# vacp2p/zerokit

Measured on AMD Instinct MI355X. Metric: RLN Groth16 proofs/sec (BN254, h=20), higher is better.
Workload: dtype u32 limbs (256-bit Montgomery integers, BN254 Fr/Fq; 8x32 and 9x29 forms)

## Files before the change

zerokit_amd/csrc/fq29.h:

```cpp
#pragma once
#include <hip/hip_runtime.h>
#include <stdint.h>

#include "curve.h"
#include "fq29_constants.h"

namespace rlnamd {

template <class C, class Mont>
struct F29 {
  uint32_t v[9];

  static constexpr uint32_t M = (1u << 29) - 1;

  static __device__ __forceinline__ F29 from_const(const uint32_t (&c)[9]) {
    F29 r;
#pragma unroll
    for (int j = 0; j < 9; j++) r.v[j] = c[j];
    return r;
  }
  static __device__ __forceinline__ F29 zero() {
    F29 r;
#pragma unroll
    for (int j = 0; j < 9; j++) r.v[j] = 0;
// ... 175 lines not shown
    const bool ge = borrow == 0;
    const uint32_t r0 = ge ? d[0] : v[0], r1 = ge ? d[1] : v[1], r2 = ge ? d[2] : v[2], r3 = ge ? d[3] : v[3],
                   r4 = ge ? d[4] : v[4], r5 = ge ? d[5] : v[5], r6 = ge ? d[6] : v[6], r7 = ge ? d[7] : v[7],
                   r8 = ge ? d[8] : v[8];
    Mont o;
    o.v[0] = r0 | (r1 << 29);
    o.v[1] = (r1 >> 3) | (r2 << 26);
    o.v[2] = (r2 >> 6) | (r3 << 23);
    o.v[3] = (r3 >> 9) | (r4 << 20);
    o.v[4] = (r4 >> 12) | (r5 << 17);
    o.v[5] = (r5 >> 15) | (r6 << 14);
    o.v[6] = (r6 >> 18) | (r7 << 11);
    o.v[7] = (r7 >> 21) | (r8 << 8);
    return o;
  }
  static __device__ __forceinline__ F29 from_fq(const Mont& a) {
    return mul(slice(a), from_const(C::FROM_FQ));
  }
  __device__ __forceinline__ Mont to_fq() const {
    return mul(*this, from_const(C::TO_FQ)).pack_reduced();
  }
  static __device__ __forceinline__ Mont mul_mont(const Mont& a, const F29& w29) { return mul(slice(a), w29).pack_reduced(); }
};

using Fq29 = F29<Fq29C, Fq>;
using Fr29 = F29<Fr29C, Fr>;

struct G1Affine29 {
  uint32_t x[8], y[8];
  __device__ __forceinline__ bool is_inf() const {
// ... 48 lines not shown
  __device__ __forceinline__ void store_xyzz(G1XYZZ* dst) const { *dst = to_xyzz(); }
  static __device__ __forceinline__ G1Acc29 load_xyzz(const G1XYZZ* src) { return from_xyzz(*src); }
  __device__ __forceinline__ void store_lds(G1Acc29* dst) const { *dst = *this; }

  static __device__ __forceinline__ G1Acc29 inf() { return {Fq29::zero(), Fq29::zero(), Fq29::zero(), Fq29::zero()}; }
  __device__ __forceinline__ bool is_inf() const { return ZZ.limbs_all_zero(); }

  __device__ __forceinline__ G1XYZZ to_xyzz() const {
    if (is_inf()) return G1XYZZ::inf();
    return {X.to_fq(), Y.to_fq(), ZZ.to_fq(), ZZZ.to_fq()};
  }
  static __device__ __forceinline__ G1Acc29 from_xyzz(const G1XYZZ& p) {
    if (p.is_inf()) return inf();
    return {Fq29::from_fq(p.X), Fq29::from_fq(p.Y), Fq29::from_fq(p.ZZ), Fq29::from_fq(p.ZZZ)};
  }

  static __device__ __forceinline__ G1Acc29 dbl_affine(const Fq29& x, const Fq29& py) {
    Fq29 U;
#pragma unroll
    for (int j = 0; j < 9; j++) U.v[j] = 2 * py.v[j];
    Fq29 V = Fq29::sqr(U);
    Fq29 W = Fq29::mul(U, V);
    Fq29 S = Fq29::mul(x, V);
    Fq29 x2 = Fq29::sqr(x);
    Fq29 Mm;
#pragma unroll
    for (int j = 0; j < 9; j++) Mm.v[j] = 3 * x2.v[j];
    Mm.normalize();
    Fq29 M2 = Fq29::sqr(Mm);
    Fq29 X3;
#pragma unroll
    for (int j = 0; j < 9; j++) X3.v[j] = M2.v[j] + Fq29C::K4T[j] - 2 * S.v[j];
    X3.normalize();
    Fq29 D = Fq29::sub(S, Fq29C::K6, X3);
    Fq29 nY = Fq29::neg_lazy(Fq29C::K4, py);
    return {X3, Fq29::dot2(Mm, D, nY, W), V, W};
  }

  __device__ __forceinline__ void madd(const G1Affine29& e, bool negate) {
    const Fq29 px = unpack29(e.x);
    Fq29 py = unpack29(e.y);
    if (negate) py = Fq29::neg_lazy(Fq29C::K2, py);
    if (is_inf()) {
      X = px;
      Y = py;
      Y.normalize();
      ZZ = Fq29::from_const(Fq29C::ONE);
      ZZZ = ZZ;
      return;
    }
    const Fq29 kX = Fq29::neg_lazy(Fq29C::K6, X);
// ... 12 lines not shown
    Fq29 PP = Fq29::sqr(P);
    ZZ = Fq29::mul(ZZ, PP);
    Fq29 Q = Fq29::mul(X, PP);
    Fq29 PPP = Fq29::mul(P, PP);
    ZZZ = Fq29::mul(ZZZ, PPP);
    Fq29 kT;
#pragma unroll
    for (int j = 0; j < 9; j++) kT.v[j] = Fq29C::K4T[j] - (PPP.v[j] + 2 * Q.v[j]);
    X = Fq29::sqr_add(R, &kT);
    Fq29 D;
#pragma unroll
    for (int j = 0; j < 9; j++) D.v[j] = Q.v[j] + Fq29C::K6[j] - X.v[j];
    Y = Fq29::dot2(R, D, nY, PPP);
  }

  __device__ __forceinline__ void add(const G1Acc29& o) {
    if (o.is_inf()) return;
    if (is_inf()) {
      *this = o;
      return;
    }
    const Fq29 U1 = Fq29::mul(X, o.ZZ), U2 = Fq29::mul(o.X, ZZ);
    const Fq29 S1 = Fq29::mul(Y, o.ZZZ), S2 = Fq29::mul(o.Y, ZZZ);
    const Fq29 P = Fq29::sub(U2, Fq29C::K2, U1), R = Fq29::sub(S2, Fq29C::K2, S1);
    if (P.is_zero_mod_q()) {
      add_same_x(this, &o);
      return;
    }
    const Fq29 PP = Fq29::sqr(P);
    ZZ = Fq29::mul(Fq29::mul(ZZ, o.ZZ), PP);
    const Fq29 Q = Fq29::mul(U1, PP);
    const Fq29 PPP = Fq29::mul(P, PP);
    ZZZ = Fq29::mul(Fq29::mul(ZZZ, o.ZZZ), PPP);
    Fq29 kT;
#pragma unroll
    for (int j = 0; j < 9; j++) kT.v[j] = Fq29C::K4T[j] - (PPP.v[j] + 2 * Q.v[j]);
    X = Fq29::sqr_add(R, &kT);
    Fq29 D;
#pragma unroll
    for (int j = 0; j < 9; j++) D.v[j] = Q.v[j] + Fq29C::K6[j] - X.v[j];
    const Fq29 nS1 = Fq29::neg_lazy(Fq29C::K4, S1);
// ... 230 lines not shown
  Fq2_29 X, Y, ZZ, ZZZ;
  static constexpr uint32_t LPP = O::LPP;
  static __device__ __forceinline__ G2AccT inf() {
    Fq2_29 z{Fq29::zero(), Fq29::zero()};
    return {z, z, z, z};
  }
  __device__ __forceinline__ bool is_inf() const { return ZZ.c0.limbs_all_zero() && ZZ.c1.limbs_all_zero(); }
  __device__ __forceinline__ G2XYZZ to_xyzz() const {
    if (is_inf()) return G2XYZZ::inf();
    return {X.to_fq2(), Y.to_fq2(), ZZ.to_fq2(), ZZZ.to_fq2()};
  }
  static __device__ __forceinline__ G2AccT from_xyzz(const G2XYZZ& p) {
    if (p.is_inf()) return inf();
    return {Fq2_29::from_fq2(p.X), Fq2_29::from_fq2(p.Y), Fq2_29::from_fq2(p.ZZ), Fq2_29::from_fq2(p.ZZZ)};
  }
  __device__ __forceinline__ void store_xyzz(G2XYZZ* dst) const {
    if (LPP == 1) {
      *dst = to_xyzz();
      return;
    }
    const bool o = Fq2PairOps::odd(), z = is_inf();
    const Fq2_29* const c[4] = {&X, &Y, &ZZ, &ZZZ};
    Fq2* const d[4] = {&dst->X, &dst->Y, &dst->ZZ, &dst->ZZZ};
#pragma unroll
    for (int k = 0; k < 4; k++) {
      const Fq v = z ? Fq::zero() : Fq2PairOps::pick(o, c[k]->c1, c[k]->c0).to_fq();
      *(o ? &d[k]->c1 : &d[k]->c0) = v;
    }
  }
  __device__ __forceinline__ void store_lds(G2AccT* dst) const {
// ... 44 lines not shown
#pragma unroll
    for (int j = 0; j < 9; j++) {
      X3.c0.v[j] = M2.c0.v[j] + Fq29C::K4T[j] - 2 * S.c0.v[j];
      X3.c1.v[j] = M2.c1.v[j] + Fq29C::K4T[j] - 2 * S.c1.v[j];
    }
    X3.c0.normalize();
    X3.c1.normalize();
    Fq2_29 D = Fq2_29::sub(S, Fq29C::K6, X3);
    Fq29 nM1 = Fq29::neg_lazy(Fq29C::K8, Mm.c1);
    Fq29 ny0 = Fq29::neg_lazy(Fq29C::K4, y.c0);
    Fq29 ny1 = Fq29::neg_lazy(Fq29C::K4, y.c1);
    Fq29 y0 = Fq29::dot4<true>(Mm.c0, D.c0, nM1, D.c1, W.c0, ny0, W.c1, y.c1);
    Fq29 y1 = Fq29::dot4<true>(Mm.c0, D.c1, Mm.c1, D.c0, W.c0, ny1, W.c1, ny0);
    return {X3, {y0, y1}, V, W};
  }

  __device__ __forceinline__ void madd(const G2Affine29& e, bool negate) {
    const Fq2_29 px{unpack29(e.x0), unpack29(e.x1)};
    Fq2_29 py{unpack29(e.y0), unpack29(e.y1)};
    if (negate) {
      py.c0 = Fq29::neg_lazy(Fq29C::K2, py.c0);
      py.c1 = Fq29::neg_lazy(Fq29C::K2, py.c1);
      py.c0.normalize();
      py.c1.normalize();
    }
    if (is_inf()) {
      X = px;
      Y = py;
      ZZ = {Fq29::from_const(Fq29C::ONE), Fq29::zero()};
      ZZZ = ZZ;
// ... 11 lines not shown
    ZZ = O::mul(ZZ, PP);
    Fq2_29 Q = O::mul(X, PP);
    Fq2_29 PPP = O::mul(P, PP);
    ZZZ = O::mul(ZZZ, PPP);
    Fq2_29 kT;
#pragma unroll
    for (int j = 0; j < 9; j++) {
      kT.c0.v[j] = Fq29C::K4T[j] - (PPP.c0.v[j] + 2 * Q.c0.v[j]);
      kT.c1.v[j] = Fq29C::K4T[j] - (PPP.c1.v[j] + 2 * Q.c1.v[j]);
    }
    X = O::sqr_add(R, kT);
    Fq2_29 D = Fq2_29::sub(Q, Fq29C::K6, X);
    Y = O::rd_minus_st(R, D, nY, Y, PPP);
  }

  __device__ __forceinline__ void add(const G2AccT* o) {
    if (o->is_inf()) return;
    if (is_inf()) {
      *this = *o;
      return;
    }
    Fq2_29 U1, P, S1, R;
    {
      const Fq2_29 oZZ = o->ZZ, oX = o->X;
      U1 = O::mul(X, oZZ);
      const Fq2_29 U2 = O::mul(oX, ZZ);
      P = Fq2_29::sub(U2, Fq29C::K2, U1);
    }
    asm volatile("" ::: "memory");
    {
      const Fq2_29 oZZZ = o->ZZZ, oY = o->Y;
      S1 = O::mul(Y, oZZZ);
      const Fq2_29 S2 = O::mul(oY, ZZZ);
      R = Fq2_29::sub(S2, Fq29C::K2, S1);
    }
    if (P.is_zero_mod_q()) {
      add_same_x(this, o);
      return;
    }
    asm volatile("" ::: "memory");
    {
      const Fq2_29 oZZ = o->ZZ;
      ZZ = O::mul(ZZ, oZZ);
    }
    {
      const Fq2_29 oZZZ = o->ZZZ;
      ZZZ = O::mul(ZZZ, oZZZ);
    }
    asm volatile("" ::: "memory");
    const Fq2_29 PP = O::sqr(P);
    ZZ = O::mul(ZZ, PP);
    const Fq2_29 Q = O::mul(U1, PP);
// ... 25 lines not shown
```

zerokit_amd/csrc/prover.hip:

```cpp
#include "prover.h"

#include <fcntl.h>
#include <stdlib.h>
#include <string.h>
#include <sys/stat.h>
#include <time.h>
#include <unistd.h>

#include <algorithm>
#include <atomic>
#include <chrono>
#include <deque>
#include <mutex>
#include <thread>

#include "prover_kernels.h"
#include "prover_plan.h"
#include "fq29.h"
#include "glv.h"
#include "pairing.h"
#include "poseidon.h"
#include "witness_ops.h"
#include "witness_lanes.h"
#include "witness_sched.h"
// ... 1343 lines not shown
  hipStream_t sA2 = big ? D.st[role[ROLE_QUOTIENT]] : !early ? D.sA2 : sh.g2_on_front ? D.sB2 : sA;
  const uint32_t pg = div_up(nb, 64);
  const uint32_t nbp = pg * 64;
  auto d2h = [&](void* host, const void* dev, size_t bytes, hipStream_t st) {
    if (!small && bytes % 16 == 0)
      hipLaunchKernelGGL(k_stage_in, dim3(div_up(bytes / 16, 64)), dim3(64), 0, st, (const uint4*)dev, (uint4*)host, (uint32_t)(bytes / 16));
    else
      RLN_HIP(hipMemcpyAsync(host, dev, bytes, hipMemcpyDeviceToHost, st));
  };
  auto walk1 = [&](hipStream_t st, const uint32_t* ids, uint32_t cnt) {
    if (!cnt) return;
    const uint32_t blocks = div_up(cnt, 8) * 8 * pg;
    if (!small) {
      const PairPlan pp{P1.prows.p, P1.prsid.p, P1.pchunks.p, P1.pout.p, P1.npchunks};
      const uint32_t pblocks = div_up(P1.npchunks, 8) * 8 * (2 * pg);
      hipLaunchKernelGGL((k_msm29<G1Acc29, G1Affine29, G1XYZZ, 4>), dim3(blocks + pblocks), dim3(64), 0, st, D.t1_29.p,
                         P1.rsid.p, P1.rows.p, P1.chunks.p, cnt, S.digits.p, S.part1.p, D.ws, dB, pg, D.nh, D.walk_clk.p, ids,
                         0u, pp);
    } else if (walk_lp) {
      hipLaunchKernelGGL((k_msm29<G1Acc29, G1Affine29, G1XYZZ, 4>), dim3(blocks), dim3(64), 0, st, D.t1_29.p, P1.rsid.p,
                         P1.rows.p, P1.chunks.p, cnt, S.digits.p, S.part1.p, D.ws, dB, pg, D.nh, nullptr, ids, PB);
    } else {
      hipLaunchKernelGGL((k_msm29<G1Acc29, G1Affine29, G1XYZZ, 2, true>), dim3(div_up(cnt, 64), nb), dim3(64), 0, st,
                         D.t1_29.p, P1.rsid.p, P1.rows.p, P1.chunks.p, cnt, S.digits.p, S.part1.p, D.ws, dB, PB, D.nh,
                         nullptr, ids);
    }
  };
  if (S.used) RLN_HIP(hipStreamWaitEvent(sA, S.free_event(), 0));
  if (streamed) {
    auto h2d = [&](void* dst, const uint8_t* src, size_t bytes) {
      hipLaunchKernelGGL(k_stage_in, dim3(div_up(bytes / 16, 64)), dim3(64), 0, sA, (const uint4*)src, (uint4*)dst,
// ... 168 lines not shown
  MARK(11, s2);
  if (P2.nchunks) {
    uint32_t blocks = div_up(P2.nchunks, 8) * 8 * pg;
    if (walk_lp)
      hipLaunchKernelGGL((k_msm29<G2Acc29, G2Affine29, G2XYZZ, 2>), dim3(blocks), dim3(64), 0, s2, D.t2_29.p, P2.rsid.p,
                         P2.rows.p, P2.chunks.p, P2.nchunks, S.digits2.p, S.part2.p, D.ws2, dB, pg, D.nh, nullptr, nullptr, PB);
    else if (tiny)
      hipLaunchKernelGGL((k_msm29<G2AccPair29, G2Affine29, G2XYZZ, 1, true>), dim3(div_up(2 * P2.nchunks, 64), nb), dim3(64), 0, s2,
                         D.t2_29.p, P2.rsid.p, P2.rows.p, P2.chunks.p, P2.nchunks, S.digits2.p, S.part2.p, D.ws2, dB, PB, D.nh,
                         nullptr);
    else if (small)
      hipLaunchKernelGGL((k_msm29<G2Acc29, G2Affine29, G2XYZZ, 1, true>), dim3(div_up(P2.nchunks, 64), nb), dim3(64), 0, s2,
                         D.t2_29.p, P2.rsid.p, P2.rows.p, P2.chunks.p, P2.nchunks, S.digits2.p, S.part2.p, D.ws2, dB, PB, D.nh,
                         nullptr);
    else
      hipLaunchKernelGGL((k_msm29<G2Acc29, G2Affine29, G2XYZZ, 2>), dim3(blocks), dim3(64), 0, s2, D.t2_29.p, P2.rsid.p,
                         P2.rows.p, P2.chunks.p, P2.nchunks, S.digits2.p, S.part2.p, D.ws2, dB, pg, D.nh,
                         D.walk_clk.p ? D.walk_clk.p + 2 : nullptr);
  }
  MARK(8, s2);
  if (!compact) RLN_HIP(hipEventRecord(S.evB, sB1));
  RLN_HIP(hipEventRecord(S.evB2, s2));
  hipStream_t sV = compact ? s2 : D.sV;
  hipStream_t sC = big ? D.st[role[ROLE_SUMS2]] : D.sC;
  if (S.used && !compact) {
    RLN_HIP(hipStreamWaitEvent(sC, S.free_event(), 0));
    RLN_HIP(hipStreamWaitEvent(sV, S.free_event(), 0));
  }
  if (!values_front) {
    if (streamed && !compact) RLN_HIP(hipStreamWaitEvent(sV, S.evU, 0));
    MARK(0, sV);
// ... 73 lines not shown
      hipLaunchKernelGGL(k_fin_out_ac, dim3(pg), dim3(64), 0, sAC, S.sums1.p, S.prod.p, S.affA.p, S.coords.p, S.comp.p, B, nbp);
    if (lone) {
      RLN_HIP(hipEventRecord(S.evA, sAC));
      RLN_HIP(hipStreamWaitEvent(sF, S.evA, 0));
    }
    RLN_HIP(hipStreamWaitEvent(sF, S.evV, 0));
  } else {
    if (tiny_partial) {
      sum2(s2);
      RLN_HIP(hipEventRecord(S.evB2, s2));
    }
    if (!values_front) RLN_HIP(hipEventRecord(S.evV, sV));
    if (compact) {
      hipStream_t sS1 = D.st[role[ROLE_SUMS1]];
      if (P1.ngroups)
        hipLaunchKernelGGL(k_sum_ranges<Fq>, dim3(pg, P1.ngroups), dim3(64), 0, sS1, S.part1.p, P1.groups.p, P1.ngroups,
                           S.grp1.p, B, nbp);
      hipLaunchKernelGGL(k_sum_ranges<Fq>, dim3(pg, P1.nseg), dim3(64), 0, sS1, S.grp1.p, P1.segs.p, P1.nseg, S.sums1.p, B, nbp);
      RLN_HIP(hipEventRecord(S.evB, sS1));
      MARK(9, sC);
      if (P2.ngroups)
        hipLaunchKernelGGL(k_sum_ranges<Fq2>, dim3(pg, P2.ngroups), dim3(64), 0, sC, S.part2.p, P2.groups.p, P2.ngroups,
                           S.grp2.p, B, nbp);
      hipLaunchKernelGGL(k_sum_ranges<Fq2>, dim3(pg, P2.nseg), dim3(64), 0, sC, S.grp2.p, P2.segs.p, P2.nseg, S.sums2.p, B, nbp);
      RLN_HIP(hipStreamWaitEvent(sC, S.evB, 0));
      RLN_HIP(hipStreamWaitEvent(sC, S.evV, 0));
    } else {
      RLN_HIP(hipStreamWaitEvent(sC, S.evV, 0));
      RLN_HIP(hipStreamWaitEvent(sC, S.evB, 0));
      if (tiny_partial) sum1(sC, {0, 1, 2, 3, 4, 5});
      RLN_HIP(hipStreamWaitEvent(sC, S.evB2, 0));
      MARK(9, sC);
    }
  }
  if (early || tiny_partial || compact) {
  } else if (small) {
    sum1(sC, {0, 1, 2, 3, 4, 5});
    sum2(sC);
  } else {
    if (P1.ngroups)
      hipLaunchKernelGGL(k_sum_ranges<Fq>, dim3(pg, P1.ngroups), dim3(64), 0, sC, S.part1.p, P1.groups.p, P1.ngroups,
                         S.grp1.p, B, nbp);
    if (P2.ngroups)
      hipLaunchKernelGGL(k_sum_ranges<Fq2>, dim3(pg, P2.ngroups), dim3(64), 0, sC, S.part2.p, P2.groups.p, P2.ngroups,
                         S.grp2.p, B, nbp);
    hipLaunchKernelGGL(k_sum_ranges<Fq>, dim3(pg, P1.nseg), dim3(64), 0, sC, S.grp1.p, P1.segs.p, P1.nseg, S.sums1.p, B, nbp);
    hipLaunchKernelGGL(k_sum_ranges<Fq2>, dim3(pg, P2.nseg), dim3(64), 0, sC, S.grp2.p, P2.segs.p, P2.nseg, S.sums2.p, B, nbp);
  }
  if (!early)
    hipLaunchKernelGGL(k_glv_fold, dim3(pg, 4), dim3(64), 0, sC, S.sums1.p, S.sums2.p, 3u, B, nbp, all4);
  if (mode == PROVE_PARTIAL) {
    hipLaunchKernelGGL(k_partial_out, dim3(pg, 4), dim3(64), 0, sC, S.sums1.p, S.sums2.p, S.pp_out.p, B, nbp);
    RLN_HIP(hipGetLastError());
    d2h(S.h_pp, S.pp_out.p, n * 320, sC);
  } else {
    if (!early) {
      if (mode == PROVE_FINISH)
        hipLaunchKernelGGL(k_add_partial, dim3(pg, 4), dim3(64), 0, sC, S.sums1.p, S.sums2.p, pp_p, B, nbp, all4, (const G1XYZZ*)nullptr);
      hipLaunchKernelGGL(k_fin_affine, dim3(pg, 3), dim3(64), 0, sC, S.sums1.p, S.sums2.p, S.affA.p, S.affB1.p,
                         S.affB2.p, B, nbp, all3);
      hipLaunchKernelGGL(k_fin_smul, dim3(pg, 2), dim3(64), 0, sC, S.affA.p, S.affB1.p, rs_p, S.tbl.p, S.prod.p, B,
                         nbp);
// ... 206 lines not shown
```

zerokit_amd/csrc/prover_kernels.h:

```cpp
#pragma once
#include <hip/hip_runtime.h>
#include <stdint.h>

#include <initializer_list>

#include "fq29.h"
#include "poseidon.h"
#include "prover.h"
#include "prover_desc.h"
#include "prover_plan.h"
#include "walk29.h"
#include "witness_ops.h"

namespace rlnamd {

struct CsrView {
  const uint32_t* ptr;
  const uint32_t* col;
  const Fr* coef;
};

struct TaskSel {
  uint8_t id[8];
};
// ... 41 lines not shown
__global__ void __launch_bounds__(256) k_ntt_mid(Fr* __restrict__ data, const Fr* __restrict__ tw_i,
                                                 const Fr* __restrict__ tw_f, int logn, const Fr* __restrict__ scale,
                                                 uint32_t B, uint32_t nb);
template <bool DIF>
__global__ void __launch_bounds__(256) k_ntt_edge(Fr* __restrict__ data, const Fr* __restrict__ tw, int logn, uint32_t B,
                                                  uint32_t nb);
__global__ void __launch_bounds__(256) k_recode(const Fr* __restrict__ V, const uint32_t* __restrict__ sig2node,
                                                uint32_t ns, const Fr* H, uint32_t n,
                                                const uint32_t* __restrict__ rs, WinSched ws1, WinSched ws2,
                                                int16_t* __restrict__ dig1, int16_t* __restrict__ dig2, uint32_t B,
                                                uint32_t nb, uint32_t part, uint32_t lg, uint32_t hq, uint32_t dB);

template <class A, class E>
__global__ void __launch_bounds__(256) k_table_to29(const A* __restrict__ src, E* __restrict__ dst, size_t n, uint32_t stride,
                                                    uint32_t k0, uint32_t npaired);
template <class F>
__global__ void __launch_bounds__(64) k_sum_ranges(const XYZZ<F>* __restrict__ src, const ChunkDesc* __restrict__ ranges,
                                                   uint32_t nranges, XYZZ<F>* __restrict__ dst, uint32_t B, uint32_t nb);
template <class F, class Acc>
__global__ void __launch_bounds__(SUM_TREE_LANES) k_sum_tree(const XYZZ<F>* __restrict__ part, const ChunkDesc* __restrict__ segchunks,
                                                  XYZZ<F>* __restrict__ dst, uint32_t B, uint32_t PB, TaskSel sel);
template <class F, class Acc>
__global__ void __launch_bounds__(SUM_TREE_LANES) k_sum_blocks(const XYZZ<F>* __restrict__ part, const ChunkDesc* __restrict__ segchunks,
                                                    const ChunkDesc* __restrict__ segblocks, XYZZ<F>* __restrict__ dst, uint32_t PB,
                                                    TaskSel sel);
__global__ void __launch_bounds__(64) k_glv_fold(G1XYZZ* __restrict__ sums1, G2XYZZ* __restrict__ sums2, uint32_t nseg1,
                                                 uint32_t B, uint32_t nb, TaskSel sel);
template <class F>
__global__ void __launch_bounds__(64) k_table_build(const Affine<F>* __restrict__ pts, uint32_t npts, WinSched ws,
                                                    Affine<F>* __restrict__ table, F* __restrict__ scratch);

// ... 61 lines not shown
```

zerokit_amd/csrc/prover_walks.hip:

```cpp
#include "prover_kernels.h"

#include "glv.h"
#include "walk29_impl.h"

namespace rlnamd {

template <class A, class E>
__global__ void __launch_bounds__(256) k_table_to29(const A* __restrict__ src, E* __restrict__ dst, size_t n, uint32_t stride,
                                                    uint32_t k0, uint32_t npaired) {
  size_t t = (size_t)blockIdx.x * 256 + threadIdx.x;
  if (t >= n) return;
  const uint32_t kl = (uint32_t)(t / stride), x = (uint32_t)(t % stride), k = k0 + kl;
  size_t o = t;
  if (k < npaired) o = (size_t)(kl & ~1u) * stride + 2 * (size_t)x + (kl & 1u);
  dst[o] = to_table29(src[t]);
}

template <class F>
__global__ void __launch_bounds__(64) k_sum_ranges(const XYZZ<F>* __restrict__ src, const ChunkDesc* __restrict__ ranges,
                                                   uint32_t nranges, XYZZ<F>* __restrict__ dst, uint32_t B, uint32_t nb) {
  __builtin_amdgcn_s_setprio(3);
  uint32_t p = blockIdx.x * 64 + threadIdx.x;
  uint32_t r = blockIdx.y;
  if (p >= nb || r >= nranges) return;
  ChunkDesc cd = ranges[r];
  XYZZ<F> acc = XYZZ<F>::inf();
  for (uint32_t i = cd.pt_begin; i < cd.pt_end; i++) acc.add(src[(size_t)i * B + p]);
  dst[(size_t)r * B + p] = acc;
}

template <class F> struct Acc29Of;
template <> struct Acc29Of<Fq> { typedef G1Acc29 type; };
template <> struct Acc29Of<Fq2> { typedef G2Acc29 type; };
extern __shared__ uint4 sum_tree_lds[];

template <class F, class Acc>
__global__ void __launch_bounds__(SUM_TREE_LANES) k_sum_tree(const XYZZ<F>* __restrict__ part, const ChunkDesc* __restrict__ segchunks,
                                                  XYZZ<F>* __restrict__ dst, uint32_t B, uint32_t PB, TaskSel sel) {
  constexpr uint32_t NP = SUM_TREE_LANES / Acc::LPP;
  Acc* sh = reinterpret_cast<Acc*>(sum_tree_lds);
  __builtin_amdgcn_s_setprio(3);
  const uint32_t p = blockIdx.x, sgi = sel.id[blockIdx.y], l = threadIdx.x / Acc::LPP;
  const ChunkDesc cd = segchunks[sgi];
  Acc acc = Acc::inf();
  for (uint32_t i = cd.pt_begin + l; i < cd.pt_end; i += NP) acc.add(Acc::load_xyzz(&part[(size_t)i * PB + p]));
#pragma unroll 1
  for (uint32_t stride = NP / 2; stride >= 1; stride >>= 1) {
    if (l >= stride && l < 2 * stride) acc.store_lds(&sh[l - stride]);
// ... 108 lines not shown
        lam = (x2.dbl() + x2) * di;
        x3 = lam.sqr() - Pm.x.dbl();
        y3 = lam * (Pm.x - x3) - Pm.y;
      }
      inv = inv * den;
      row[m + i - 1] = {x3, y3};
    }
    __threadfence_block();
    __syncthreads();
  }
}


template __global__ void k_table_to29<G1Affine, G1Affine29>(const G1Affine* __restrict__ src, G1Affine29* __restrict__ dst, size_t n, uint32_t stride, uint32_t k0, uint32_t npaired);
template __global__ void k_table_to29<G2Affine, G2Affine29>(const G2Affine* __restrict__ src, G2Affine29* __restrict__ dst, size_t n, uint32_t stride, uint32_t k0, uint32_t npaired);
template __global__ void k_sum_ranges<Fq>(const XYZZ<Fq>* __restrict__ src, const ChunkDesc* __restrict__ ranges, uint32_t nranges, XYZZ<Fq>* __restrict__ dst, uint32_t B, uint32_t nb);
template __global__ void k_sum_ranges<Fq2>(const XYZZ<Fq2>* __restrict__ src, const ChunkDesc* __restrict__ ranges, uint32_t nranges, XYZZ<Fq2>* __restrict__ dst, uint32_t B, uint32_t nb);
template __global__ void k_sum_tree<Fq, G1Acc29>(const XYZZ<Fq>* __restrict__ part, const ChunkDesc* __restrict__ segchunks, XYZZ<Fq>* __restrict__ dst, uint32_t B, uint32_t PB, TaskSel sel);
template __global__ void k_sum_tree<Fq, G1AccPair29>(const XYZZ<Fq>* __restrict__ part, const ChunkDesc* __restrict__ segchunks, XYZZ<Fq>* __restrict__ dst, uint32_t B, uint32_t PB, TaskSel sel);
template __global__ void k_sum_tree<Fq2, G2Acc29>(const XYZZ<Fq2>* __restrict__ part, const ChunkDesc* __restrict__ segchunks, XYZZ<Fq2>* __restrict__ dst, uint32_t B, uint32_t PB, TaskSel sel);
template __global__ void k_sum_blocks<Fq, G1Acc29>(const XYZZ<Fq>* __restrict__ part, const ChunkDesc* __restrict__ segchunks, const ChunkDesc* __restrict__ segblocks, XYZZ<Fq>* __restrict__ dst, uint32_t PB, TaskSel sel);
template __global__ void k_sum_blocks<Fq, G1AccPair29>(const XYZZ<Fq>* __restrict__ part, const ChunkDesc* __restrict__ segchunks, const ChunkDesc* __restrict__ segblocks, XYZZ<Fq>* __restrict__ dst, uint32_t PB, TaskSel sel);
template __global__ void k_sum_blocks<Fq2, G2Acc29>(const XYZZ<Fq2>* __restrict__ part, const ChunkDesc* __restrict__ segchunks, const ChunkDesc* __restrict__ segblocks, XYZZ<Fq2>* __restrict__ dst, uint32_t PB, TaskSel sel);
template __global__ void k_sum_tree<Fq2, G2AccPair29>(const XYZZ<Fq2>* __restrict__ part, const ChunkDesc* __restrict__ segchunks, XYZZ<Fq2>* __restrict__ dst, uint32_t B, uint32_t PB, TaskSel sel);
template __global__ void k_sum_blocks<Fq2, G2AccPair29>(const XYZZ<Fq2>* __restrict__ part, const ChunkDesc* __restrict__ segchunks, const ChunkDesc* __restrict__ segblocks, XYZZ<Fq2>* __restrict__ dst, uint32_t PB, TaskSel sel);
template __global__ void k_table_build<Fq>(const Affine<Fq>* __restrict__ pts, uint32_t npts, WinSched ws, Affine<Fq>* __restrict__ table, Fq* __restrict__ scratch);
template __global__ void k_table_build<Fq2>(const Affine<Fq2>* __restrict__ pts, uint32_t npts, WinSched ws, Affine<Fq2>* __restrict__ table, Fq2* __restrict__ scratch);
template __global__ void k_msm29<G1Acc29, G1Affine29, G1XYZZ, 4, false>(const G1Affine29* __restrict__ table, const uint32_t* __restrict__ sid, const uint32_t* __restrict__ rows, const ChunkDesc* __restrict__ chunks, uint32_t nchunks, const int16_t* __restrict__ digits, G1XYZZ* __restrict__ part, WinSched ws, uint32_t B, uint32_t pgroups, uint32_t nh, unsigned long long* __restrict__ clk, const uint32_t* __restrict__ chunk_ids, uint32_t pstride, PairPlan pairs);
template __global__ void k_msm29<G1Acc29, G1Affine29, G1XYZZ, 2, true>(const G1Affine29* __restrict__ table, const uint32_t* __restrict__ sid, const uint32_t* __restrict__ rows, const ChunkDesc* __restrict__ chunks, uint32_t nchunks, const int16_t* __restrict__ digits, G1XYZZ* __restrict__ part, WinSched ws, uint32_t B, uint32_t pgroups, uint32_t nh, unsigned long long* __restrict__ clk, const uint32_t* __restrict__ chunk_ids, uint32_t pstride, PairPlan pairs);
template __global__ void k_msm29<G2Acc29, G2Affine29, G2XYZZ, 2, false>(const G2Affine29* __restrict__ table, const uint32_t* __restrict__ sid, const uint32_t* __restrict__ rows, const ChunkDesc* __restrict__ chunks, uint32_t nchunks, const int16_t* __restrict__ digits, G2XYZZ* __restrict__ part, WinSched ws, uint32_t B, uint32_t pgroups, uint32_t nh, unsigned long long* __restrict__ clk, const uint32_t* __restrict__ chunk_ids, uint32_t pstride, PairPlan pairs);
template __global__ void k_msm29<G2Acc29, G2Affine29, G2XYZZ, 1, true>(const G2Affine29* __restrict__ table, const uint32_t* __restrict__ sid, const uint32_t* __restrict__ rows, const ChunkDesc* __restrict__ chunks, uint32_t nchunks, const int16_t* __restrict__ digits, G2XYZZ* __restrict__ part, WinSched ws, uint32_t B, uint32_t pgroups, uint32_t nh, unsigned long long* __restrict__ clk, const uint32_t* __restrict__ chunk_ids, uint32_t pstride, PairPlan pairs);
template __global__ void k_msm29<G2AccPair29, G2Affine29, G2XYZZ, 1, true>(const G2Affine29* __restrict__ table, const uint32_t* __restrict__ sid, const uint32_t* __restrict__ rows, const ChunkDesc* __restrict__ chunks, uint32_t nchunks, const int16_t* __restrict__ digits, G2XYZZ* __restrict__ part, WinSched ws, uint32_t B, uint32_t pgroups, uint32_t nh, unsigned long long* __restrict__ clk, const uint32_t* __restrict__ chunk_ids, uint32_t pstride, PairPlan pairs);

}
```

zerokit_amd/csrc/walk29.h:

```cpp
#pragma once
#include <hip/hip_runtime.h>
#include <stdint.h>

#include "fq29.h"
#include "prover_desc.h"

namespace rlnamd {

template <class Entry>
__device__ __forceinline__ const Entry* row_base(const Entry* __restrict__ table, uint32_t roww, uint32_t stride, uint32_t* shift) {
  const uint32_t k = roww & ROW_INDEX, il = (roww >> 30) & 1u;
  *shift = il;
  return table + (size_t)(il ? (k & ~1u) : k) * stride + (il ? (k & 1u) : 0u);
}

struct PairPlan {
  const uint32_t* rows;
  const uint32_t* sid;
  const ChunkDesc* chunks;
  const uint32_t* out;
  uint32_t nchunks;
};

template <class Acc, class Entry, class Out, int WAVES, bool LANECHUNK = false>
__global__ void __launch_bounds__(64) __attribute__((amdgpu_waves_per_eu(WAVES, WAVES))) k_msm29(const Entry* __restrict__ table, const uint32_t* __restrict__ sid,
                                              const uint32_t* __restrict__ rows, const ChunkDesc* __restrict__ chunks,
                                              uint32_t nchunks, const int16_t* __restrict__ digits,
                                              Out* __restrict__ part, WinSched ws, uint32_t B, uint32_t pgroups,
                                              uint32_t nh, unsigned long long* __restrict__ clk,
                                              const uint32_t* __restrict__ chunk_ids = nullptr, uint32_t pstride = 0,
                                              PairPlan pairs = PairPlan{nullptr, nullptr, nullptr, nullptr, 0});

}
```

zerokit_amd/csrc/walk29_impl.h:

```cpp
#pragma once
#include "walk29.h"

namespace rlnamd {

template <class Acc, class Entry, class Out, int WAVES, bool LANECHUNK>
__global__ void __launch_bounds__(64) __attribute__((amdgpu_waves_per_eu(WAVES, WAVES))) k_msm29(const Entry* __restrict__ table, const uint32_t* __restrict__ sid,
                                              const uint32_t* __restrict__ rows, const ChunkDesc* __restrict__ chunks,
                                              uint32_t nchunks, const int16_t* __restrict__ digits,
                                              Out* __restrict__ part, WinSched ws, uint32_t B, uint32_t pgroups,
                                              uint32_t nh, unsigned long long* __restrict__ clk,
                                              const uint32_t* __restrict__ chunk_ids, uint32_t pstride, PairPlan pairs) {
  const unsigned long long c0 = clk ? clock64() : 0, w0 = clk ? wall_clock64() : 0;
  uint32_t L = blockIdx.x;
  const int W = ws.W;
  if (LANECHUNK) {
    const uint32_t idx = (L * 64 + threadIdx.x) / Acc::LPP, p = blockIdx.y;
    if (idx >= nchunks) return;
    const uint32_t chunk = chunk_ids ? chunk_ids[idx] : idx;
    const ChunkDesc cd = chunks[chunk];
    Acc acc = Acc::inf();
    struct Cur {
      uint32_t i, j;
    };
    auto adv = [&](Cur& c) {
// ... 55 lines not shown
#pragma unroll 1
  for (uint32_t i = cd.pt_begin; i < cd.pt_end; i++) {
    const uint32_t kk = R[i] + member;
    const int16_t* dg = digits + ((size_t)S[i] * nh + (kk >> 31)) * W * B + p;
    uint32_t sh;
    const Entry* row = row_base(table, kk, ws.stride, &sh);
#pragma unroll 1
    for (int j = 0; j < W; j++) {
      int d = dg[(size_t)j * B];
      if (d != 0) {
        uint32_t e = (uint32_t)(d < 0 ? -d : d) - 1;
        acc.madd(row[(size_t)(ws.ro[j] + e) << sh], d < 0);
      }
    }
  }
  part[(size_t)out_slot * (pstride ? pstride : B) + p] = acc.to_xyzz();
  if (clk && threadIdx.x == 0 && (L & 63) == 0) {
    atomicAdd(clk, clock64() - c0);
    atomicAdd(clk + 1, wall_clock64() - w0);
  }
}

}
```

Measured before the change: 23120.

## Hand off MSM partials in loose 29-bit Montgomery form to range-sum kernels

The MSM walk kernels now write bucket partials in a loosely reduced, packed 9x29-limb form instead of fully converting each coordinate back to canonical 8x32 Montgomery with a multiply. The range-sum kernels are reworked to accumulate with the 29-bit accumulator types, slicing the handoff form directly, and only the final segment pass converts to canonical XYZZ. This removes per-partial to_fq/from_fq multiplies and replaces 32-bit XYZZ adds with the faster 29-bit adds. The same-x case is handled inline with a new doubling routine. It relies on loose values fitting in 256 bits after a conditional 4q subtraction on X, and adds LDS staging for G2 operands.

```diff
diff --git a/zerokit_amd/csrc/fq29.h b/zerokit_amd/csrc/fq29.h
--- a/zerokit_amd/csrc/fq29.h
+++ b/zerokit_amd/csrc/fq29.h
@@ -213,6 +213,30 @@
     o.v[7] = (r7 >> 21) | (r8 << 8);
     return o;
   }
+  __device__ __forceinline__ Mont pack_loose() const {
+    Mont o;
+    o.v[0] = v[0] | (v[1] << 29);
+    o.v[1] = (v[1] >> 3) | (v[2] << 26);
+    o.v[2] = (v[2] >> 6) | (v[3] << 23);
+    o.v[3] = (v[3] >> 9) | (v[4] << 20);
+    o.v[4] = (v[4] >> 12) | (v[5] << 17);
+    o.v[5] = (v[5] >> 15) | (v[6] << 14);
+    o.v[6] = (v[6] >> 18) | (v[7] << 11);
+    o.v[7] = (v[7] >> 21) | (v[8] << 8);
+    return o;
+  }
+  __device__ __forceinline__ F29 minus_4q_if_above() const {
+    const bool above = v[8] > C::KP[4][8];
+    F29 r;
+    int32_t borrow = 0;
+#pragma unroll
+    for (int j = 0; j < 9; j++) {
+      const int32_t x = (int32_t)v[j] - (int32_t)(above ? C::KP[4][j] : 0u) + borrow;
+      r.v[j] = j < 8 ? (uint32_t)x & M : (uint32_t)x;
+      borrow = x >> 29;
+    }
+    return r;
+  }
   static __device__ __forceinline__ F29 from_fq(const Mont& a) {
     return mul(slice(a), from_const(C::FROM_FQ));
   }
@@ -291,6 +315,12 @@
     if (p.is_inf()) return inf();
     return {Fq29::from_fq(p.X), Fq29::from_fq(p.Y), Fq29::from_fq(p.ZZ), Fq29::from_fq(p.ZZZ)};
   }
+  __device__ __forceinline__ void store_handoff(G1XYZZ* dst) const {
+    *dst = {X.minus_4q_if_above().pack_loose(), Y.pack_loose(), ZZ.pack_loose(), ZZZ.pack_loose()};
+  }
+  static __device__ __forceinline__ G1Acc29 from_handoff(const G1XYZZ& p) {
+    return {Fq29::slice(p.X), Fq29::slice(p.Y), Fq29::slice(p.ZZ), Fq29::slice(p.ZZZ)};
+  }
 
   static __device__ __forceinline__ G1Acc29 dbl_affine(const Fq29& x, const Fq29& py) {
     Fq29 U;
@@ -312,6 +342,12 @@
     Fq29 D = Fq29::sub(S, Fq29C::K6, X3);
     Fq29 nY = Fq29::neg_lazy(Fq29C::K4, py);
     return {X3, Fq29::dot2(Mm, D, nY, W), V, W};
+  }
+  __device__ __forceinline__ G1Acc29 dbl() const {
+    G1Acc29 r = dbl_affine(X, Y);
+    r.ZZ = Fq29::mul(r.ZZ, ZZ);
+    r.ZZZ = Fq29::mul(r.ZZZ, ZZZ);
+    return r;
   }
 
   __device__ __forceinline__ void madd(const G1Affine29& e, bool negate) {
@@ -354,6 +390,7 @@
     Y = Fq29::dot2(R, D, nY, PPP);
   }
 
+  template <bool SAME_X_HERE = false>
   __device__ __forceinline__ void add(const G1Acc29& o) {
     if (o.is_inf()) return;
     if (is_inf()) {
@@ -364,7 +401,12 @@
     const Fq29 S1 = Fq29::mul(Y, o.ZZZ), S2 = Fq29::mul(o.Y, ZZZ);
     const Fq29 P = Fq29::sub(U2, Fq29C::K2, U1), R = Fq29::sub(S2, Fq29C::K2, S1);
     if (P.is_zero_mod_q()) {
-      add_same_x(this, &o);
+      if (!SAME_X_HERE)
+        add_same_x(this, &o);
+      else if (R.is_zero_mod_q())
+        *this = dbl();
+      else
+        *this = inf();
       return;
     }
     const Fq29 PP = Fq29::sqr(P);
@@ -625,6 +667,16 @@
     if (p.is_inf()) return inf();
     return {Fq2_29::from_fq2(p.X), Fq2_29::from_fq2(p.Y), Fq2_29::from_fq2(p.ZZ), Fq2_29::from_fq2(p.ZZZ)};
   }
+  __device__ __forceinline__ void store_handoff(G2XYZZ* dst) const {
+    *dst = {{X.c0.minus_4q_if_above().pack_loose(), X.c1.minus_4q_if_above().pack_loose()},
+            {Y.c0.pack_loose(), Y.c1.pack_loose()},
+            {ZZ.c0.pack_loose(), ZZ.c1.pack_loose()},
+            {ZZZ.c0.pack_loose(), ZZZ.c1.pack_loose()}};
+  }
+  static __device__ __forceinline__ G2AccT from_handoff(const G2XYZZ& p) {
+    return {{Fq29::slice(p.X.c0), Fq29::slice(p.X.c1)}, {Fq29::slice(p.Y.c0), Fq29::slice(p.Y.c1)},
+            {Fq29::slice(p.ZZ.c0), Fq29::slice(p.ZZ.c1)}, {Fq29::slice(p.ZZZ.c0), Fq29::slice(p.ZZZ.c1)}};
+  }
   __device__ __forceinline__ void store_xyzz(G2XYZZ* dst) const {
     if (LPP == 1) {
       *dst = to_xyzz();
@@ -699,6 +751,12 @@
     Fq29 y1 = Fq29::dot4<true>(Mm.c0, D.c1, Mm.c1, D.c0, W.c0, ny1, W.c1, ny0);
     return {X3, {y0, y1}, V, W};
   }
+  __device__ __forceinline__ G2AccT dbl() const {
+    G2AccT r = dbl_affine(X, Y);
+    r.ZZ = Fq2_29::mul(r.ZZ, ZZ);
+    r.ZZZ = Fq2_29::mul(r.ZZZ, ZZZ);
+    return r;
+  }
 
   __device__ __forceinline__ void madd(const G2Affine29& e, bool negate) {
     const Fq2_29 px{unpack29(e.x0), unpack29(e.x1)};
@@ -740,6 +798,7 @@
     Y = O::rd_minus_st(R, D, nY, Y, PPP);
   }
 
+  template <bool SAME_X_HERE = false>
   __device__ __forceinline__ void add(const G2AccT* o) {
     if (o->is_inf()) return;
     if (is_inf()) {
@@ -761,7 +820,12 @@
       R = Fq2_29::sub(S2, Fq29C::K2, S1);
     }
     if (P.is_zero_mod_q()) {
-      add_same_x(this, o);
+      if (!SAME_X_HERE)
+        add_same_x(this, o);
+      else if (R.is_zero_mod_q())
+        *this = dbl();
+      else
+        *this = inf();
       return;
     }
     asm volatile("" ::: "memory");
diff --git a/zerokit_amd/csrc/prover.hip b/zerokit_amd/csrc/prover.hip
--- a/zerokit_amd/csrc/prover.hip
+++ b/zerokit_amd/csrc/prover.hip
@@ -1381,7 +1381,7 @@
     if (!small) {
       const PairPlan pp{P1.prows.p, P1.prsid.p, P1.pchunks.p, P1.pout.p, P1.npchunks};
       const uint32_t pblocks = div_up(P1.npchunks, 8) * 8 * (2 * pg);
-      hipLaunchKernelGGL((k_msm29<G1Acc29, G1Affine29, G1XYZZ, 4>), dim3(blocks + pblocks), dim3(64), 0, st, D.t1_29.p,
+      hipLaunchKernelGGL((k_msm29<G1Acc29, G1Affine29, G1XYZZ, 4, false, TAIL_HANDOFF>), dim3(blocks + pblocks), dim3(64), 0, st, D.t1_29.p,
                          P1.rsid.p, P1.rows.p, P1.chunks.p, cnt, S.digits.p, S.part1.p, D.ws, dB, pg, D.nh, D.walk_clk.p, ids,
                          0u, pp);
     } else if (walk_lp) {
@@ -1580,7 +1580,7 @@
                          D.t2_29.p, P2.rsid.p, P2.rows.p, P2.chunks.p, P2.nchunks, S.digits2.p, S.part2.p, D.ws2, dB, PB, D.nh,
                          nullptr);
     else
-      hipLaunchKernelGGL((k_msm29<G2Acc29, G2Affine29, G2XYZZ, 2>), dim3(blocks), dim3(64), 0, s2, D.t2_29.p, P2.rsid.p,
+      hipLaunchKernelGGL((k_msm29<G2Acc29, G2Affine29, G2XYZZ, 2, false, TAIL_HANDOFF_NO_STRIDE>), dim3(blocks), dim3(64), 0, s2, D.t2_29.p, P2.rsid.p,
                          P2.rows.p, P2.chunks.p, P2.nchunks, S.digits2.p, S.part2.p, D.ws2, dB, pg, D.nh,
                          D.walk_clk.p ? D.walk_clk.p + 2 : nullptr);
   }
@@ -1684,15 +1684,15 @@
     if (compact) {
       hipStream_t sS1 = D.st[role[ROLE_SUMS1]];
       if (P1.ngroups)
-        hipLaunchKernelGGL(k_sum_ranges<Fq>, dim3(pg, P1.ngroups), dim3(64), 0, sS1, S.part1.p, P1.groups.p, P1.ngroups,
+        hipLaunchKernelGGL((k_sum_ranges<Fq, false>), dim3(pg, P1.ngroups), dim3(64), 0, sS1, S.part1.p, P1.groups.p, P1.ngroups,
                            S.grp1.p, B, nbp);
-      hipLaunchKernelGGL(k_sum_ranges<Fq>, dim3(pg, P1.nseg), dim3(64), 0, sS1, S.grp1.p, P1.segs.p, P1.nseg, S.sums1.p, B, nbp);
+      hipLaunchKernelGGL((k_sum_ranges<Fq, true>), dim3(pg, P1.nseg), dim3(64), 0, sS1, S.grp1.p, P1.segs.p, P1.nseg, S.sums1.p, B, nbp);
       RLN_HIP(hipEventRecord(S.evB, sS1));
       MARK(9, sC);
       if (P2.ngroups)
-        hipLaunchKernelGGL(k_sum_ranges<Fq2>, dim3(pg, P2.ngroups), dim3(64), 0, sC, S.part2.p, P2.groups.p, P2.ngroups,
+        hipLaunchKernelGGL((k_sum_ranges<Fq2, false>), dim3(pg, P2.ngroups), dim3(64), 0, sC, S.part2.p, P2.groups.p, P2.ngroups,
                            S.grp2.p, B, nbp);
-      hipLaunchKernelGGL(k_sum_ranges<Fq2>, dim3(pg, P2.nseg), dim3(64), 0, sC, S.grp2.p, P2.segs.p, P2.nseg, S.sums2.p, B, nbp);
+      hipLaunchKernelGGL((k_sum_ranges<Fq2, true>), dim3(pg, P2.nseg), dim3(64), 0, sC, S.grp2.p, P2.segs.p, P2.nseg, S.sums2.p, B, nbp);
       RLN_HIP(hipStreamWaitEvent(sC, S.evB, 0));
       RLN_HIP(hipStreamWaitEvent(sC, S.evV, 0));
     } else {
@@ -1709,13 +1709,13 @@
     sum2(sC);
   } else {
     if (P1.ngroups)
-      hipLaunchKernelGGL(k_sum_ranges<Fq>, dim3(pg, P1.ngroups), dim3(64), 0, sC, S.part1.p, P1.groups.p, P1.ngroups,
+      hipLaunchKernelGGL((k_sum_ranges<Fq, false>), dim3(pg, P1.ngroups), dim3(64), 0, sC, S.part1.p, P1.groups.p, P1.ngroups,
                          S.grp1.p, B, nbp);
     if (P2.ngroups)
-      hipLaunchKernelGGL(k_sum_ranges<Fq2>, dim3(pg, P2.ngroups), dim3(64), 0, sC, S.part2.p, P2.groups.p, P2.ngroups,
+      hipLaunchKernelGGL((k_sum_ranges<Fq2, false>), dim3(pg, P2.ngroups), dim3(64), 0, sC, S.part2.p, P2.groups.p, P2.ngroups,
                          S.grp2.p, B, nbp);
-    hipLaunchKernelGGL(k_sum_ranges<Fq>, dim3(pg, P1.nseg), dim3(64), 0, sC, S.grp1.p, P1.segs.p, P1.nseg, S.sums1.p, B, nbp);
-    hipLaunchKernelGGL(k_sum_ranges<Fq2>, dim3(pg, P2.nseg), dim3(64), 0, sC, S.grp2.p, P2.segs.p, P2.nseg, S.sums2.p, B, nbp);
+    hipLaunchKernelGGL((k_sum_ranges<Fq, true>), dim3(pg, P1.nseg), dim3(64), 0, sC, S.grp1.p, P1.segs.p, P1.nseg, S.sums1.p, B, nbp);
+    hipLaunchKernelGGL((k_sum_ranges<Fq2, true>), dim3(pg, P2.nseg), dim3(64), 0, sC, S.grp2.p, P2.segs.p, P2.nseg, S.sums2.p, B, nbp);
   }
   if (!early)
     hipLaunchKernelGGL(k_glv_fold, dim3(pg, 4), dim3(64), 0, sC, S.sums1.p, S.sums2.p, 3u, B, nbp, all4);
diff --git a/zerokit_amd/csrc/prover_kernels.h b/zerokit_amd/csrc/prover_kernels.h
--- a/zerokit_amd/csrc/prover_kernels.h
+++ b/zerokit_amd/csrc/prover_kernels.h
@@ -79,7 +79,7 @@
 template <class A, class E>
 __global__ void __launch_bounds__(256) k_table_to29(const A* __restrict__ src, E* __restrict__ dst, size_t n, uint32_t stride,
                                                     uint32_t k0, uint32_t npaired);
-template <class F>
+template <class F, bool LAST>
 __global__ void __launch_bounds__(64) k_sum_ranges(const XYZZ<F>* __restrict__ src, const ChunkDesc* __restrict__ ranges,
                                                    uint32_t nranges, XYZZ<F>* __restrict__ dst, uint32_t B, uint32_t nb);
 template <class F, class Acc>
diff --git a/zerokit_amd/csrc/prover_walks.hip b/zerokit_amd/csrc/prover_walks.hip
--- a/zerokit_amd/csrc/prover_walks.hip
+++ b/zerokit_amd/csrc/prover_walks.hip
@@ -16,22 +16,32 @@
   dst[o] = to_table29(src[t]);
 }
 
-template <class F>
+template <class F> struct Acc29Of;
+template <> struct Acc29Of<Fq> { typedef G1Acc29 type; };
+template <> struct Acc29Of<Fq2> { typedef G2Acc29 type; };
+
+__device__ __forceinline__ void add_handoff(G1Acc29& acc, const G1XYZZ* src) { acc.add<true>(G1Acc29::from_handoff(*src)); }
+__device__ __forceinline__ void add_handoff(G2Acc29& acc, const G2XYZZ* src) {
+  __shared__ G2Acc29 operand[64];
+  operand[threadIdx.x] = G2Acc29::from_handoff(*src);
+  acc.add<true>(&operand[threadIdx.x]);
+}
+
+template <class F, bool LAST>
 __global__ void __launch_bounds__(64) k_sum_ranges(const XYZZ<F>* __restrict__ src, const ChunkDesc* __restrict__ ranges,
                                                    uint32_t nranges, XYZZ<F>* __restrict__ dst, uint32_t B, uint32_t nb) {
+  typedef typename Acc29Of<F>::type Acc;
   __builtin_amdgcn_s_setprio(3);
   uint32_t p = blockIdx.x * 64 + threadIdx.x;
   uint32_t r = blockIdx.y;
   if (p >= nb || r >= nranges) return;
   ChunkDesc cd = ranges[r];
-  XYZZ<F> acc = XYZZ<F>::inf();
-  for (uint32_t i = cd.pt_begin; i < cd.pt_end; i++) acc.add(src[(size_t)i * B + p]);
-  dst[(size_t)r * B + p] = acc;
-}
-
-template <class F> struct Acc29Of;
-template <> struct Acc29Of<Fq> { typedef G1Acc29 type; };
-template <> struct Acc29Of<Fq2> { typedef G2Acc29 type; };
+  Acc acc = Acc::inf();
+  for (uint32_t i = cd.pt_begin; i < cd.pt_end; i++) add_handoff(acc, &src[(size_t)i * B + p]);
+  XYZZ<F>* const out = &dst[(size_t)r * B + p];
+  if (LAST) *out = acc.to_xyzz(); else acc.store_handoff(out);
+}
+
 extern __shared__ uint4 sum_tree_lds[];
 
 template <class F, class Acc>
@@ -170,8 +180,10 @@
 
 template __global__ void k_table_to29<G1Affine, G1Affine29>(const G1Affine* __restrict__ src, G1Affine29* __restrict__ dst, size_t n, uint32_t stride, uint32_t k0, uint32_t npaired);
 template __global__ void k_table_to29<G2Affine, G2Affine29>(const G2Affine* __restrict__ src, G2Affine29* __restrict__ dst, size_t n, uint32_t stride, uint32_t k0, uint32_t npaired);
-template __global__ void k_sum_ranges<Fq>(const XYZZ<Fq>* __restrict__ src, const ChunkDesc* __restrict__ ranges, uint32_t nranges, XYZZ<Fq>* __restrict__ dst, uint32_t B, uint32_t nb);
-template __global__ void k_sum_ranges<Fq2>(const XYZZ<Fq2>* __restrict__ src, const ChunkDesc* __restrict__ ranges, uint32_t nranges, XYZZ<Fq2>* __restrict__ dst, uint32_t B, uint32_t nb);
+template __global__ void k_sum_ranges<Fq, false>(const XYZZ<Fq>* __restrict__ src, const ChunkDesc* __restrict__ ranges, uint32_t nranges, XYZZ<Fq>* __restrict__ dst, uint32_t B, uint32_t nb);
+template __global__ void k_sum_ranges<Fq, true>(const XYZZ<Fq>* __restrict__ src, const ChunkDesc* __restrict__ ranges, uint32_t nranges, XYZZ<Fq>* __restrict__ dst, uint32_t B, uint32_t nb);
+template __global__ void k_sum_ranges<Fq2, false>(const XYZZ<Fq2>* __restrict__ src, const ChunkDesc* __restrict__ ranges, uint32_t nranges, XYZZ<Fq2>* __restrict__ dst, uint32_t B, uint32_t nb);
+template __global__ void k_sum_ranges<Fq2, true>(const XYZZ<Fq2>* __restrict__ src, const ChunkDesc* __restrict__ ranges, uint32_t nranges, XYZZ<Fq2>* __restrict__ dst, uint32_t B, uint32_t nb);
 template __global__ void k_sum_tree<Fq, G1Acc29>(const XYZZ<Fq>* __restrict__ part, const ChunkDesc* __restrict__ segchunks, XYZZ<Fq>* __restrict__ dst, uint32_t B, uint32_t PB, TaskSel sel);
 template __global__ void k_sum_tree<Fq, G1AccPair29>(const XYZZ<Fq>* __restrict__ part, const ChunkDesc* __restrict__ segchunks, XYZZ<Fq>* __restrict__ dst, uint32_t B, uint32_t PB, TaskSel sel);
 template __global__ void k_sum_tree<Fq2, G2Acc29>(const XYZZ<Fq2>* __restrict__ part, const ChunkDesc* __restrict__ segchunks, XYZZ<Fq2>* __restrict__ dst, uint32_t B, uint32_t PB, TaskSel sel);
@@ -183,8 +195,10 @@
 template __global__ void k_table_build<Fq>(const Affine<Fq>* __restrict__ pts, uint32_t npts, WinSched ws, Affine<Fq>* __restrict__ table, Fq* __restrict__ scratch);
 template __global__ void k_table_build<Fq2>(const Affine<Fq2>* __restrict__ pts, uint32_t npts, WinSched ws, Affine<Fq2>* __restrict__ table, Fq2* __restrict__ scratch);
 template __global__ void k_msm29<G1Acc29, G1Affine29, G1XYZZ, 4, false>(const G1Affine29* __restrict__ table, const uint32_t* __restrict__ sid, const uint32_t* __restrict__ rows, const ChunkDesc* __restrict__ chunks, uint32_t nchunks, const int16_t* __restrict__ digits, G1XYZZ* __restrict__ part, WinSched ws, uint32_t B, uint32_t pgroups, uint32_t nh, unsigned long long* __restrict__ clk, const uint32_t* __restrict__ chunk_ids, uint32_t pstride, PairPlan pairs);
+template __global__ void k_msm29<G1Acc29, G1Affine29, G1XYZZ, 4, false, TAIL_HANDOFF>(const G1Affine29* __restrict__ table, const uint32_t* __restrict__ sid, const uint32_t* __restrict__ rows, const ChunkDesc* __restrict__ chunks, uint32_t nchunks, const int16_t* __restrict__ digits, G1XYZZ* __restrict__ part, WinSched ws, uint32_t B, uint32_t pgroups, uint32_t nh, unsigned long long* __restrict__ clk, const uint32_t* __restrict__ chunk_ids, uint32_t pstride, PairPlan pairs);
 template __global__ void k_msm29<G1Acc29, G1Affine29, G1XYZZ, 2, true>(const G1Affine29* __restrict__ table, const uint32_t* __restrict__ sid, const uint32_t* __restrict__ rows, const ChunkDesc* __restrict__ chunks, uint32_t nchunks, const int16_t* __restrict__ digits, G1XYZZ* __restrict__ part, WinSched ws, uint32_t B, uint32_t pgroups, uint32_t nh, unsigned long long* __restrict__ clk, const uint32_t* __restrict__ chunk_ids, uint32_t pstride, PairPlan pairs);
 template __global__ void k_msm29<G2Acc29, G2Affine29, G2XYZZ, 2, false>(const G2Affine29* __restrict__ table, const uint32_t* __restrict__ sid, const uint32_t* __restrict__ rows, const ChunkDesc* __restrict__ chunks, uint32_t nchunks, const int16_t* __restrict__ digits, G2XYZZ* __restrict__ part, WinSched ws, uint32_t B, uint32_t pgroups, uint32_t nh, unsigned long long* __restrict__ clk, const uint32_t* __restrict__ chunk_ids, uint32_t pstride, PairPlan pairs);
+template __global__ void k_msm29<G2Acc29, G2Affine29, G2XYZZ, 2, false, TAIL_HANDOFF_NO_STRIDE>(const G2Affine29* __restrict__ table, const uint32_t* __restrict__ sid, const uint32_t* __restrict__ rows, const ChunkDesc* __restrict__ chunks, uint32_t nchunks, const int16_t* __restrict__ digits, G2XYZZ* __restrict__ part, WinSched ws, uint32_t B, uint32_t pgroups, uint32_t nh, unsigned long long* __restrict__ clk, const uint32_t* __restrict__ chunk_ids, uint32_t pstride, PairPlan pairs);
 template __global__ void k_msm29<G2Acc29, G2Affine29, G2XYZZ, 1, true>(const G2Affine29* __restrict__ table, const uint32_t* __restrict__ sid, const uint32_t* __restrict__ rows, const ChunkDesc* __restrict__ chunks, uint32_t nchunks, const int16_t* __restrict__ digits, G2XYZZ* __restrict__ part, WinSched ws, uint32_t B, uint32_t pgroups, uint32_t nh, unsigned long long* __restrict__ clk, const uint32_t* __restrict__ chunk_ids, uint32_t pstride, PairPlan pairs);
 template __global__ void k_msm29<G2AccPair29, G2Affine29, G2XYZZ, 1, true>(const G2Affine29* __restrict__ table, const uint32_t* __restrict__ sid, const uint32_t* __restrict__ rows, const ChunkDesc* __restrict__ chunks, uint32_t nchunks, const int16_t* __restrict__ digits, G2XYZZ* __restrict__ part, WinSched ws, uint32_t B, uint32_t pgroups, uint32_t nh, unsigned long long* __restrict__ clk, const uint32_t* __restrict__ chunk_ids, uint32_t pstride, PairPlan pairs);
 
diff --git a/zerokit_amd/csrc/walk29.h b/zerokit_amd/csrc/walk29.h
--- a/zerokit_amd/csrc/walk29.h
+++ b/zerokit_amd/csrc/walk29.h
@@ -22,7 +22,8 @@
   uint32_t nchunks;
 };
 
-template <class Acc, class Entry, class Out, int WAVES, bool LANECHUNK = false>
+enum : int { TAIL_XYZZ = 0, TAIL_HANDOFF = 1, TAIL_HANDOFF_NO_STRIDE = 2 };
+template <class Acc, class Entry, class Out, int WAVES, bool LANECHUNK = false, int TAIL = TAIL_XYZZ>
 __global__ void __launch_bounds__(64) __attribute__((amdgpu_waves_per_eu(WAVES, WAVES))) k_msm29(const Entry* __restrict__ table, const uint32_t* __restrict__ sid,
                                               const uint32_t* __restrict__ rows, const ChunkDesc* __restrict__ chunks,
                                               uint32_t nchunks, const int16_t* __restrict__ digits,
diff --git a/zerokit_amd/csrc/walk29_impl.h b/zerokit_amd/csrc/walk29_impl.h
--- a/zerokit_amd/csrc/walk29_impl.h
+++ b/zerokit_amd/csrc/walk29_impl.h
@@ -3,7 +3,7 @@
 
 namespace rlnamd {
 
-template <class Acc, class Entry, class Out, int WAVES, bool LANECHUNK>
+template <class Acc, class Entry, class Out, int WAVES, bool LANECHUNK, int TAIL>
 __global__ void __launch_bounds__(64) __attribute__((amdgpu_waves_per_eu(WAVES, WAVES))) k_msm29(const Entry* __restrict__ table, const uint32_t* __restrict__ sid,
                                               const uint32_t* __restrict__ rows, const ChunkDesc* __restrict__ chunks,
                                               uint32_t nchunks, const int16_t* __restrict__ digits,
@@ -93,7 +93,8 @@
       }
     }
   }
-  part[(size_t)out_slot * (pstride ? pstride : B) + p] = acc.to_xyzz();
+  Out* const dst = &part[(size_t)out_slot * (pstride ? pstride : B) + p];
+  if (TAIL == TAIL_HANDOFF || (TAIL == TAIL_HANDOFF_NO_STRIDE && !pstride)) acc.store_handoff(dst); else *dst = acc.to_xyzz();
   if (clk && threadIdx.x == 0 && (L & 63) == 0) {
     atomicAdd(clk, clock64() - c0);
     atomicAdd(clk + 1, wall_clock64() - w0);
```

New measurement: 23120. No clear change (-0.0%).
